# helenypzhang/Subspace-Multimodal-Learning

Measured on AMD Instinct MI355X. Metric: bags/sec fwd+bwd, DeformCrossTransMIL N=10k x 512, higher is better.
Workload: dtype f32

## Files before the change

include/smml.h:

```cpp
#ifndef SMML_H_
#define SMML_H_

#include <stddef.h>

#ifdef __cplusplus
extern "C" {
#endif

const char* smml_last_error(void);
int smml_abi_version(void);
int smml_device_check(int device);
void* smml_event_create(void);
int smml_event_destroy(void* ev);
int smml_event_record(void* ev, void* stream);
int smml_event_elapsed_ms(void* start, void* stop, float* ms);

int smml_gemm_f32(const float* A, const float* B, float* C, const float* bias, const float* residual,
                  int M, int N, int K, long long sam, long long sak, long long sbk, long long sbn,
                  long long ldc, long long ldr, int nb0, int nb1, long long sa0, long long sa1,
                  long long sb0, long long sb1, long long sc0, long long sc1, long long sbias0,
                  long long sbias1, int bias_mode, int rows_per_bias, long long bias_ld, int act,
                  int splitk, int accumulate, float alpha, float beta, void* stream);
void smml_gemm_force_generic(int on);
void smml_gemm_set_mode(int mode);
int smml_gemm_get_mode(void);
void smml_gemm_set_small_tile(int v);

int smml_gemm_b16(const void* A, const void* B, void* C, const float* bias, int M, int N, int K, long long lda, long long ldb,
                  long long ldc, int trans, int out_bf16, int splitk, void* stream);
void smml_gemm_b16_set_tile(int mode);
void smml_gemm_b16_set_slice_major(int on);
int smml_gemm_b16_batched(const void* A, const void* B, void* C, const float* bias, int M, int N, int K, long long lda, long long ldb,
                          long long ldc, int trans, int out_bf16, int splitk, int nb, long long sa, long long sb, long long sc, void* stream);

int smml_layernorm_fwd_f32(const float* x, const float* gamma, const float* beta, float* y, float* mean,
                           float* rstd, long long R, int C, float eps, void* stream);
int smml_layernorm_bwd_f32(const float* x, const float* dy, const float* gamma, const float* mean,
                           const float* rstd, float* dx, float* dgamma, float* dbeta, long long R, int C,
                           long long rows_per_dy, float dy_scale, int accumulate_dx, void* stream);

int smml_colsum_f32(const float* x, float* out, int nb, long long R, int C, float scale, void* stream);

int smml_orth_loss_f32(const float* P, const float* Ph, const float* G, const float* Gh, const float* dloss, float* loss,
                       float* dP, float* dPh, float* dG, float* dGh, int B, int D, float gamma, void* stream);

int smml_batchloss_tail_f32(const float* go, const float* gv, const float* dloss, float* loss, float* dgo, float* dgv, int R, int nv,
                            float n_total, void* stream);

int smml_relu_bwd_f32(const float* dy, const float* y, float* dx, long long n, void* stream);

int smml_offsets_out_len(int s, int ks, int r);
int smml_offsets_fwd_f32(const float* q, const float* w0, const float* b0, const float* w2, float* vgrid,
                         float* vs, int B, int Hh, int Ww, int G, int dg, int ks, int r, int posdim,
                         float offset_scale, void* stream);
size_t smml_offsets_bwd_workspace_bytes(int B, int Hh, int Ww, int G, int dg, int ks, int r, int posdim);
// ... 208 lines not shown
```

subspace-multimodal-learning_amd/_capi.py:

```python
from __future__ import annotations

import ctypes as C
import os
from typing import Optional

import torch

_PKG = os.path.dirname(os.path.abspath(__file__))
LIB_PATH = os.environ.get("SMML_LIB") or os.path.join(_PKG, "lib", "libsmml_hip.so")

_f = C.c_void_p


class DeformOpts(C.Structure):
    _fields_ = [("seed_offset", C.c_void_p), ("raw_distance", C.c_int), ("mask_table", C.c_void_p), ("mask_table_pmax", C.c_float),
                ("export_masks", C.c_void_p), ("region_lds_cap", C.c_int)]


_o = C.POINTER(DeformOpts)
_i, _ll, _fl, _sz = C.c_int, C.c_longlong, C.c_float, C.c_size_t

ABI_VERSION = 2

SIGNATURES = {
    "smml_last_error": (C.c_char_p, []),
    "smml_abi_version": (_i, []),
    "smml_device_check": (_i, [_i]),
    "smml_gemm_f32": (_i, [_f, _f, _f, _f, _f, _i, _i, _i, _ll, _ll, _ll, _ll, _ll, _ll, _i, _i, _ll, _ll, _ll, _ll,
                           _ll, _ll, _ll, _ll, _i, _i, _ll, _i, _i, _i, _fl, _fl, _f]),
    "smml_gemm_force_generic": (None, [_i]),
    "smml_gemm_set_mode": (None, [_i]),
    "smml_gemm_get_mode": (_i, []),
    "smml_gemm_set_small_tile": (None, [_i]),
    "smml_gemm_b16": (_i, [_f, _f, _f, _f, _i, _i, _i, _ll, _ll, _ll, _i, _i, _i, _f]),
    "smml_gemm_b16_set_tile": (None, [_i]),
    "smml_gemm_b16_set_slice_major": (None, [_i]),
    "smml_gemm_b16_batched": (_i, [_f, _f, _f, _f, _i, _i, _i, _ll, _ll, _ll, _i, _i, _i, _i, _ll, _ll, _ll, _f]),
    "smml_attn16_fwd_workspace_bytes": (_sz, [_i, _i, _i]),
    "smml_attn16_fwd_f32": (_i, [_f, _f, _f, _f, _f, _f, _sz, _i, _i, _i, _i, _fl, _i, _i, _i, _f]),
    "smml_attn16_set_fewkeys": (None, [_i]),
    "smml_attn16_set_query_blocks": (None, [_i]),
    "smml_attn16_fwd_b16": (_i, [_f, _f, _f, _f, _f, _f, _f, _sz, _i, _i, _i, _i, _fl, _i, _ll, _ll, _ll, _ll, _ll, _ll, _f]),
    "smml_attn16_bwd_b16": (_i, [_f] * 11 + [_sz, _i, _i, _i, _i, _fl, _i] + [_ll] * 9 + [_i, _f]),
    "smml_attn16_bwd_workspace_bytes": (_sz, [_i, _i, _i]),
    "smml_attn16_bwd_f32": (_i, [_f] * 10 + [_f, _sz, _i, _i, _i, _i, _fl, _i, _i, _f]),
    "smml_layernorm_fwd_f32": (_i, [_f, _f, _f, _f, _f, _f, _ll, _i, _fl, _f]),
    "smml_layernorm_bwd_f32": (_i, [_f, _f, _f, _f, _f, _f, _f, _f, _ll, _i, _ll, _fl, _i, _f]),
    "smml_colsum_f32": (_i, [_f, _f, _i, _ll, _i, _fl, _f]),
    "smml_orth_loss_f32": (_i, [_f] * 10 + [_i, _i, _fl, _f]),
    "smml_batchloss_tail_f32": (_i, [_f, _f, _f, _f, _f, _f, _i, _i, _fl, _f]),
    "smml_relu_bwd_f32": (_i, [_f, _f, _f, _ll, _f]),
    "smml_offsets_out_len": (_i, [_i, _i, _i]),
    "smml_offsets_fwd_f32": (_i, [_f, _f, _f, _f, _f, _f, _i, _i, _i, _i, _i, _i, _i, _i, _fl, _f]),
    "smml_offsets_bwd_workspace_bytes": (_sz, [_i, _i, _i, _i, _i, _i, _i, _i]),
    "smml_offsets_bwd_f32": (_i, [_f, _f, _f, _f, _f, _f, _f, _f, _f, _f, _f, _sz, _i, _i, _i, _i, _i, _i, _i, _i, _fl, _i, _f]),
    "smml_bilinear_sample_fwd_f32": (_i, [_f, _f, _f, _i, _i, _i, _i, _i, _i, _i, _f]),
    "smml_bilinear_sample_bwd_f32": (_i, [_f, _f, _f, _f, _f, _i, _i, _i, _i, _i, _i, _i, _f]),
    "smml_bilinear_corners_f32": (_i, [_f, _f, _f, _f, _i, _i, _i, _i, _f]),
    "smml_deform_attn_nst": (_i, [_i]),
    "smml_deform_attn_fwd_f32": (_i, [_f] * 15 + [_i, _i, _i, _i, _i, _i, _fl, _fl, C.c_ulonglong, _f, _f, _f] + [_o]),
    "smml_deform_attn_dropout_mask_f32": (_i, [_f, _i, _i, _i, _i, _fl, C.c_ulonglong, _f] + [_o]),
    "smml_deform_attn_relu1_masks": (_i, [_f, _f, _f, _f, _f, _i, _i, _i, _i, _i, _f] + [_o]),
# ... 118 lines not shown
```

subspace-multimodal-learning_amd/csrc/gemm.hip:

```cpp
#include "smml_common.h"
#include <atomic>

namespace {

constexpr int BM = 128, BN = 64, BK = 16;
constexpr int LDA = BM + 4, LDB = BN + 4;

struct GemmArgs {
  const float* A; const float* B; float* C; const float* bias; const float* residual;
  int M, N, K;
  long long sam, sak, sbk, sbn, ldc, ldr;
  int nb0, nb1;
  long long sa0, sa1, sb0, sb1, sc0, sc1, sbias0, sbias1;
  int bias_mode, rows_per_bias; long long bias_ld;
  int act, splitk; float alpha, beta;
  int atomic;
  int swap_xy;
};

__device__ __forceinline__ float apply_act(float v, int act) {
  if (act == 1) return fmaxf(v, 0.f);
  if (act == 2) return tanhf(v);
  return v;
}

__global__ __launch_bounds__(256) void gemm_f32_kernel(GemmArgs g) {
  __shared__ float As[BK][LDA];
  __shared__ float Bs[BK][LDB];
  const int tid = threadIdx.x, wave = tid >> 6, lane = tid & 63, c = lane & 31, hf = lane >> 5;
  const int zb = blockIdx.z / g.splitk, ks = blockIdx.z - zb * g.splitk;
  const int b0 = zb / g.nb1, b1 = zb - b0 * g.nb1;
  const float* A = g.A + b0 * g.sa0 + b1 * g.sa1;
  const float* B = g.B + b0 * g.sb0 + b1 * g.sb1;
  float* C = g.C + b0 * g.sc0 + b1 * g.sc1;
  const int m0 = (g.swap_xy ? blockIdx.y : blockIdx.x) * BM, n0 = (g.swap_xy ? blockIdx.x : blockIdx.y) * BN;
  const int ktiles = (g.K + BK - 1) / BK;
  const int tps = (ktiles + g.splitk - 1) / g.splitk;
  const int kt0 = ks * tps, kt1 = min(ktiles, kt0 + tps);

  floatx16 acc0 = {0}, acc1 = {0};
  const bool a_kcontig = (g.sak == 1);
  const bool b_kcontig = (g.sbk == 1) && (g.sbn != 1);

  for (int kt = kt0; kt < kt1; ++kt) {
    const int k0 = kt * BK;
    __syncthreads();
    if (a_kcontig) {
      const int k = tid & 15;
#pragma unroll
      for (int i = 0; i < 8; ++i) {
// ... 30 lines not shown
    __syncthreads();
#pragma unroll
    for (int st = 0; st < BK / 2; ++st) {
      const float a = As[2 * st + hf][wave * 32 + c];
      acc0 = mfma32(a, Bs[2 * st + hf][c], acc0);
      acc1 = mfma32(a, Bs[2 * st + hf][32 + c], acc1);
    }
  }

  const float* bias = g.bias ? g.bias + b0 * g.sbias0 + b1 * g.sbias1 : nullptr;
  const float* res = g.residual ? g.residual + b0 * g.sc0 + b1 * g.sc1 : nullptr;
#pragma unroll
  for (int t = 0; t < 2; ++t) {
    const int n = n0 + 32 * t + c;
    if (n >= g.N) continue;
#pragma unroll
    for (int r = 0; r < 16; ++r) {
      const int m = m0 + wave * 32 + acc_row(r, hf);
      if (m >= g.M) continue;
      float v = g.alpha * (t == 0 ? acc0[r] : acc1[r]);
      if (g.atomic) {
        if (bias && ks == 0) v += (g.bias_mode == 2) ? bias[(m / g.rows_per_bias) * g.bias_ld + n] : bias[n];
        atomicAdd(&C[m * g.ldc + n], v);
      } else {
        if (bias) v += (g.bias_mode == 2) ? bias[(m / g.rows_per_bias) * g.bias_ld + n] : bias[n];
        v = apply_act(v, g.act);
        if (res) v = fmaf(g.beta, res[m * g.ldr + n], v);
        C[m * g.ldc + n] = v;
      }
    }
  }
}

template <int BN_, bool A_KC, bool B_KC, int FBM = 128>
__global__ __launch_bounds__(256, 2) void gemm_f32_fast_kernel(GemmArgs g) {
  constexpr int FBK = 16, NI = BN_ / 64, MI = FBM / 64;
  constexpr int NA = FBM / 64;
  constexpr int A_LD = A_KC ? (FBK + 4) : (FBM + 4);
  constexpr int B_LD = B_KC ? (FBK + 4) : (BN_ + 4);
  __shared__ __attribute__((aligned(16))) float As[(A_KC ? FBM : FBK) * A_LD];
  __shared__ __attribute__((aligned(16))) float Bs[(B_KC ? BN_ : FBK) * B_LD];
  const int tid = threadIdx.x, wave = tid >> 6, lane = tid & 63, c = lane & 31, hf = lane >> 5;
  const int wm = wave >> 1, wn = wave & 1;
  const int zb = blockIdx.z / g.splitk, ks = blockIdx.z - zb * g.splitk;
  const int b0 = zb / g.nb1, b1 = zb - b0 * g.nb1;
  const float* A = g.A + b0 * g.sa0 + b1 * g.sa1;
  const float* B = g.B + b0 * g.sb0 + b1 * g.sb1;
  float* C = g.C + b0 * g.sc0 + b1 * g.sc1;
  const int m0 = (g.swap_xy ? blockIdx.y : blockIdx.x) * FBM, n0 = (g.swap_xy ? blockIdx.x : blockIdx.y) * BN_;
  const int ktiles = (g.K + FBK - 1) / FBK;
  const int tps = (ktiles + g.splitk - 1) / g.splitk;
  const int kt0 = ks * tps, kt1 = min(ktiles, kt0 + tps);

  float4 ra[NA], rb[NI];
  const float* pa[NA];
  const float* pb[NI];
  int ka[NA], kb_[NI];
  int fa[NA], fb[NI];
  constexpr int MQ = FBM / 4;
#pragma unroll
  for (int i = 0; i < NA; ++i) {
    if (A_KC) {
      const int row = (tid >> 2) + 64 * i, kq = tid & 3;
      pa[i] = A + (long long)min(m0 + row, g.M - 1) * g.sam + 4 * kq;
      ka[i] = 4 * kq; fa[i] = 1;
    } else {
      const int idx = tid + 256 * i, k = idx / MQ, mq = idx - k * MQ, gm = m0 + 4 * mq;
      pa[i] = A + min(gm, g.M - 1);
      ka[i] = k; fa[i] = (gm >= g.M) ? 0 : (gm + 3 < g.M ? 1 : 2);
    }
  }
#pragma unroll
  for (int i = 0; i < NI; ++i) {
    if (B_KC) {
      const int row = (tid >> 2) + 64 * i, kq = tid & 3;
      pb[i] = B + (long long)min(n0 + row, g.N - 1) * g.sbn + 4 * kq;
      kb_[i] = 4 * kq; fb[i] = 1;
    } else {
      constexpr int NQ = BN_ / 4;
      const int idx = tid + 256 * i, k = idx / NQ, nq = idx - k * NQ, gn = n0 + 4 * nq;
      pb[i] = B + min(gn, g.N - 1);
      kb_[i] = k; fb[i] = (gn >= g.N) ? 0 : (gn + 3 < g.N ? 1 : 2);
    }
  }
  auto load_tile = [&](int kt) {
    const int k0 = kt * FBK;
#pragma unroll
    for (int i = 0; i < NA; ++i) {
      if (A_KC) {
        ra[i] = (k0 + ka[i] < g.K) ? *reinterpret_cast<const float4*>(pa[i] + k0) : make_float4(0.f, 0.f, 0.f, 0.f);
      } else {
        const int k = k0 + ka[i];
        const float* p = pa[i] + (long long)min(k, g.K - 1) * g.sak;
        if (k >= g.K || fa[i] == 0) ra[i] = make_float4(0.f, 0.f, 0.f, 0.f);
        else if (fa[i] == 1) ra[i] = *reinterpret_cast<const float4*>(p);
        else { const int gm = m0 + 4 * ((tid + 256 * i) % MQ), last = g.M - 1 - gm;
               ra[i] = make_float4(p[0], p[min(1, last)], p[min(2, last)], p[min(3, last)]); }
      }
    }
#pragma unroll
    for (int i = 0; i < NI; ++i) {
      if (B_KC) {
        rb[i] = (k0 + kb_[i] < g.K) ? *reinterpret_cast<const float4*>(pb[i] + k0) : make_float4(0.f, 0.f, 0.f, 0.f);
      } else {
        const int k = k0 + kb_[i];
        const float* p = pb[i] + (long long)min(k, g.K - 1) * g.sbk;
        if (k >= g.K || fb[i] == 0) rb[i] = make_float4(0.f, 0.f, 0.f, 0.f);
        else if (fb[i] == 1) rb[i] = *reinterpret_cast<const float4*>(p);
        else { constexpr int NQ = BN_ / 4; const int idx = tid + 256 * i, gn = n0 + 4 * (idx - (idx / NQ) * NQ), last = g.N - 1 - gn;
               rb[i] = make_float4(p[0], p[min(1, last)], p[min(2, last)], p[min(3, last)]); }
      }
    }
  };
  auto store_tile = [&]() {
#pragma unroll
    for (int i = 0; i < NA; ++i) {
      if (A_KC) { const int row = (tid >> 2) + 64 * i, kq = tid & 3; *reinterpret_cast<float4*>(&As[row * A_LD + 4 * kq]) = ra[i]; }
      else { const int idx = tid + 256 * i, k = idx / MQ, mq = idx - k * MQ; *reinterpret_cast<float4*>(&As[k * A_LD + 4 * mq]) = ra[i]; }
    }
#pragma unroll
    for (int i = 0; i < NI; ++i) {
      if (B_KC) { const int row = (tid >> 2) + 64 * i, kq = tid & 3; *reinterpret_cast<float4*>(&Bs[row * B_LD + 4 * kq]) = rb[i]; }
      else { constexpr int NQ = BN_ / 4; const int idx = tid + 256 * i, k = idx / NQ, nq = idx - k * NQ;
             *reinterpret_cast<float4*>(&Bs[k * B_LD + 4 * nq]) = rb[i]; }
    }
  };

  floatx16 acc[MI][NI];
#pragma unroll
  for (int mi = 0; mi < MI; ++mi)
#pragma unroll
    for (int ni = 0; ni < NI; ++ni) acc[mi][ni] = floatx16{0};

  if (kt0 < kt1) load_tile(kt0);
  for (int kt = kt0; kt < kt1; ++kt) {
    __syncthreads();
    store_tile();
    __syncthreads();
    if (kt + 1 < kt1) load_tile(kt + 1);
    float af[MI][8], bf[NI][8];
#pragma unroll
    for (int mi = 0; mi < MI; ++mi) {
      const int row = wm * (FBM / 2) + mi * 32 + c;
      if (A_KC) {
        const float4 x = *reinterpret_cast<const float4*>(&As[row * A_LD + 8 * hf]);
        const float4 y = *reinterpret_cast<const float4*>(&As[row * A_LD + 8 * hf + 4]);
        af[mi][0] = x.x; af[mi][1] = x.y; af[mi][2] = x.z; af[mi][3] = x.w;
        af[mi][4] = y.x; af[mi][5] = y.y; af[mi][6] = y.z; af[mi][7] = y.w;
      } else {
#pragma unroll
        for (int st = 0; st < 8; ++st) af[mi][st] = As[(8 * hf + st) * A_LD + row];
      }
    }
#pragma unroll
    for (int ni = 0; ni < NI; ++ni) {
      const int col = wn * (BN_ / 2) + ni * 32 + c;
      if (B_KC) {
        const float4 x = *reinterpret_cast<const float4*>(&Bs[col * B_LD + 8 * hf]);
        const float4 y = *reinterpret_cast<const float4*>(&Bs[col * B_LD + 8 * hf + 4]);
        bf[ni][0] = x.x; bf[ni][1] = x.y; bf[ni][2] = x.z; bf[ni][3] = x.w;
        bf[ni][4] = y.x; bf[ni][5] = y.y; bf[ni][6] = y.z; bf[ni][7] = y.w;
      } else {
#pragma unroll
        for (int st = 0; st < 8; ++st) bf[ni][st] = Bs[(8 * hf + st) * B_LD + col];
      }
    }
#pragma unroll
    for (int st = 0; st < 8; ++st)
#pragma unroll
      for (int mi = 0; mi < MI; ++mi)
#pragma unroll
        for (int ni = 0; ni < NI; ++ni) acc[mi][ni] = mfma32(af[mi][st], bf[ni][st], acc[mi][ni]);
  }

  const float* bias = g.bias ? g.bias + b0 * g.sbias0 + b1 * g.sbias1 : nullptr;
  const float* res = g.residual ? g.residual + b0 * g.sc0 + b1 * g.sc1 : nullptr;
  if (!g.atomic && m0 + FBM <= g.M && n0 + BN_ <= g.N) {
#pragma unroll
    for (int mi = 0; mi < MI; ++mi)
#pragma unroll
      for (int ni = 0; ni < NI; ++ni) {
        const int n = n0 + wn * (BN_ / 2) + ni * 32 + c;
        const int mb = m0 + wm * (FBM / 2) + mi * 32;
        float rv[16];
#pragma unroll
        for (int r = 0; r < 16; ++r) rv[r] = res ? res[(long long)(mb + acc_row(r, hf)) * g.ldr + n] : 0.f;
#pragma unroll
        for (int r = 0; r < 16; ++r) {
          const int m = mb + acc_row(r, hf);
          float v = g.alpha * acc[mi][ni][r];
          if (bias) v += (g.bias_mode == 2) ? bias[(m / g.rows_per_bias) * g.bias_ld + n] : bias[n];
          v = apply_act(v, g.act);
          C[(long long)m * g.ldc + n] = fmaf(g.beta, rv[r], v);
        }
      }
    return;
  }
#pragma unroll
  for (int mi = 0; mi < MI; ++mi)
#pragma unroll
    for (int ni = 0; ni < NI; ++ni) {
      const int n = n0 + wn * (BN_ / 2) + ni * 32 + c;
      if (n >= g.N) continue;
#pragma unroll
      for (int r = 0; r < 16; ++r) {
// ... 199 lines not shown
  for (int mi = 0; mi < MI; ++mi)
#pragma unroll
    for (int ni = 0; ni < NI; ++ni) {
      const int n = n0 + wn * (BN_ / 2) + ni * 32 + c;
      if (n >= g.N) continue;
#pragma unroll
      for (int r = 0; r < 16; ++r) {
        const int m = m0 + wm * (FBM / 2) + mi * 32 + acc_row(r, hf);
        if (m >= g.M) continue;
        float v = g.alpha * acc[mi][ni][r];
        if (g.atomic) {
          if (bias && ks == 0) v += (g.bias_mode == 2) ? bias[(m / g.rows_per_bias) * g.bias_ld + n] : bias[n];
          atomicAdd(&C[m * g.ldc + n], v);
        } else {
          if (bias) v += (g.bias_mode == 2) ? bias[(m / g.rows_per_bias) * g.bias_ld + n] : bias[n];
          v = apply_act(v, g.act);
          if (res) v = fmaf(g.beta, res[m * g.ldr + n], v);
          C[m * g.ldc + n] = v;
        }
      }
    }
}

}

static std::atomic<int> g_force_generic{0};
static std::atomic<int> g_mode{0};
extern "C" void smml_gemm_force_generic(int on) { g_force_generic = on; }
extern "C" void smml_gemm_set_mode(int mode) { g_mode = mode; }
extern "C" int smml_gemm_get_mode(void) { return g_mode; }
static std::atomic<int> g_small_tile{0};
extern "C" void smml_gemm_set_small_tile(int v) { g_small_tile = v; }

extern "C" int smml_gemm_f32(const float* A, const float* B, float* C, const float* bias, const float* residual,
                             int M, int N, int K, long long sam, long long sak, long long sbk, long long sbn,
                             long long ldc, long long ldr, int nb0, int nb1, long long sa0, long long sa1,
                             long long sb0, long long sb1, long long sc0, long long sc1, long long sbias0,
                             long long sbias1, int bias_mode, int rows_per_bias, long long bias_ld, int act,
                             int splitk, int accumulate, float alpha, float beta, void* stream) {
  SMML_REQUIRE(A && B && C, "smml_gemm_f32: null operand");
  SMML_REQUIRE(M > 0 && N > 0 && K > 0 && nb0 > 0 && nb1 > 0, "smml_gemm_f32: non-positive size (M=%d N=%d K=%d)", M, N, K);
  SMML_REQUIRE(splitk >= 1, "smml_gemm_f32: splitk must be >= 1");
  const int atomic = (splitk > 1 || accumulate) ? 1 : 0;
  SMML_REQUIRE(!(atomic && (act != 0 || residual)), "smml_gemm_f32: split-K / accumulate excludes activation/residual");
  SMML_REQUIRE(bias_mode >= 0 && bias_mode <= 2, "smml_gemm_f32: bad bias_mode %d", bias_mode);
  SMML_REQUIRE(bias_mode != 2 || rows_per_bias > 0, "smml_gemm_f32: rows_per_bias must be positive");
  SMML_REQUIRE(act >= 0 && act <= 2, "smml_gemm_f32: bad activation %d", act);
  const long long gz = (long long)nb0 * nb1 * splitk;
  const long long gy = (N + BN - 1) / BN, gx = (M + BM - 1) / BM;
  const int swap_xy = gy > 65535;
  SMML_REQUIRE(gz <= 65535 && (swap_xy ? gx : gy) <= 65535,
               "smml_gemm_f32: grid too large (batch*splitk=%lld, row tiles=%lld, col tiles=%lld)", gz, gx, gy);
  GemmArgs g{A, B, C, bias_mode ? bias : nullptr, residual, M, N, K, sam, sak, sbk, sbn, ldc, ldr, nb0, nb1,
             sa0, sa1, sb0, sb1, sc0, sc1, sbias0, sbias1, bias_mode, rows_per_bias > 0 ? rows_per_bias : 1,
             bias_ld, act, splitk, alpha, beta, atomic, swap_xy};
  SMML_REQUIRE(!bias_mode || bias, "smml_gemm_f32: bias_mode set but bias is null");
  auto al4 = [](long long v) { return (v & 3) == 0; };
  auto al16 = [](const void* p) { return (((size_t)p) & 15) == 0; };
  const bool a_kc = (sak == 1), a_mc = (sam == 1 && sak != 1);
  const bool b_kc = (sbk == 1 && sbn != 1), b_nc = (sbn == 1);
  const bool a_ok = al16(A) && al4(sa0) && al4(sa1) && ((a_kc && al4(sam)) || (a_mc && al4(sak)));
  const bool b_ok = al16(B) && al4(sb0) && al4(sb1) && ((b_kc && al4(sbn)) || (b_nc && al4(sbk)));
  const bool k_ok = (!a_kc && !b_kc) || (K % 4) == 0;
  if (a_ok && b_ok && k_ok && !g_force_generic) {
    const int bn = (N > 64 && gx * ((N + 127) / 128) * gz >= 1024) ? 128 : 64;
    const long long fy = (N + bn - 1) / bn;
    const bool small = bn == 64 && M > 64 && (g_small_tile == 2 || (g_small_tile == 0 && gx * fy * gz < 512));
    const long long fx = small ? (M + 63) / 64 : gx;
    const int fswap = fy > 65535;
    SMML_REQUIRE((fswap ? fx : fy) <= 65535, "smml_gemm_f32: grid too large");
    g.swap_xy = fswap;
    dim3 grid((unsigned)(fswap ? fy : fx), (unsigned)(fswap ? fx : fy), (unsigned)gz);
    hipStream_t st = (hipStream_t)stream;
    const bool bf3 = (g_mode == 2) || (g_mode == 0 && K >= 2048 && M >= 1024 && N >= 1024);
    const bool bf1 = (g_mode == 3), f1 = (g_mode == 4);
#define SMML_FAST(BNV, AK, BK2)                                                                   \
  do {                                                                                            \
    if (f1) hipLaunchKernelGGL((gemm_bf3_kernel<BNV, AK, BK2, 1, 128, true>), grid, dim3(256), 0, st, g); \
    else if (bf1) hipLaunchKernelGGL((gemm_bf3_kernel<BNV, AK, BK2, 1>), grid, dim3(256), 0, st, g);   \
    else if (bf3) hipLaunchKernelGGL((gemm_bf3_kernel<BNV, AK, BK2>), grid, dim3(256), 0, st, g); \
    else hipLaunchKernelGGL((gemm_f32_fast_kernel<BNV, AK, BK2>), grid, dim3(256), 0, st, g);     \
  } while (0)
#define SMML_SMALL(AK, BK2)                                                                          \
  do {                                                                                               \
    if (f1) hipLaunchKernelGGL((gemm_bf3_kernel<64, AK, BK2, 1, 64, true>), grid, dim3(256), 0, st, g);   \
    else if (bf1) hipLaunchKernelGGL((gemm_bf3_kernel<64, AK, BK2, 1, 64>), grid, dim3(256), 0, st, g);   \
    else if (bf3) hipLaunchKernelGGL((gemm_bf3_kernel<64, AK, BK2, 3, 64>), grid, dim3(256), 0, st, g); \
    else hipLaunchKernelGGL((gemm_f32_fast_kernel<64, AK, BK2, 64>), grid, dim3(256), 0, st, g);     \
  } while (0)
    if (small) {
      if (a_kc && b_kc) SMML_SMALL(true, true); else if (a_kc) SMML_SMALL(true, false);
      else if (b_kc) SMML_SMALL(false, true); else SMML_SMALL(false, false);
    } else if (bn == 128) {
      if (a_kc && b_kc) SMML_FAST(128, true, true); else if (a_kc) SMML_FAST(128, true, false);
      else if (b_kc) SMML_FAST(128, false, true); else SMML_FAST(128, false, false);
    } else {
      if (a_kc && b_kc) SMML_FAST(64, true, true); else if (a_kc) SMML_FAST(64, true, false);
      else if (b_kc) SMML_FAST(64, false, true); else SMML_FAST(64, false, false);
    }
#undef SMML_FAST
#undef SMML_SMALL
    SMML_LAUNCH_CHECK("smml_gemm_f32/fast");
    return SMML_OK;
  }
  dim3 grid((unsigned)(swap_xy ? gy : gx), (unsigned)(swap_xy ? gx : gy), (unsigned)gz);
  hipLaunchKernelGGL(gemm_f32_kernel, grid, dim3(256), 0, (hipStream_t)stream, g);
  SMML_LAUNCH_CHECK("smml_gemm_f32");
  return SMML_OK;
}
```

subspace-multimodal-learning_amd/functional.py:

```python
from __future__ import annotations

import math
import os
from typing import Optional

import ctypes as C_

import torch

from . import _capi as capi

ACT_NONE, ACT_RELU, ACT_TANH = 0, 1, 2


class KernelTimer:

    def __init__(self):
        self.enabled = False
        self.pairs = {"deform_attn_fwd": [], "cpb_bwd": []}
        self.work = {"deform_attn_fwd": [], "cpb_bwd": []}

    def events(self, name, pairs_count):
        if not self.enabled:
            return None, None
# ... 56 lines not shown
            n *= d
        if (n == 0 or n > self.LIMIT or torch.device(device).type != "cuda" or not self.enabled
                or torch.cuda.is_current_stream_capturing()):
            return torch.zeros(shape, device=device, dtype=torch.float32)
        key = torch.device(device).index if torch.device(device).index is not None else torch.cuda.current_device()
        buf, used = self.slabs.get(key, (None, self.SLAB))
        n4 = (n + 3) & ~3
        if used + n4 > self.SLAB:
            buf, used = torch.zeros(self.SLAB, device=device, dtype=torch.float32), 0
        self.slabs[key] = (buf, used + n4)
        return buf[used:used + n].view(shape)


_ZEROS = _ZeroPool()


def _zeros_like(t: torch.Tensor) -> torch.Tensor:
    return _ZEROS.zeros(t.shape, t.device)


def _c(t: torch.Tensor) -> torch.Tensor:
    if t.dtype != torch.float32:
        t = t.float()
    return t if t.is_contiguous() else t.contiguous()


def _gemm(A, B, C, *, M, N, K, sam, sak, sbk, sbn, ldc, bias=None, bias_mode=0, rows_per_bias=1, bias_ld=0,
          residual=None, ldr=0, act=ACT_NONE, splitk=1, alpha=1.0, nb0=1, nb1=1, sa0=0, sa1=0, sb0=0, sb1=0,
          sc0=0, sc1=0, sbias0=0, sbias1=0, beta=1.0, accumulate=0):
    capi.check(capi.lib().smml_gemm_f32(
        capi.fptr(A), capi.fptr(B), capi.fptr(C), capi.fptr(bias), capi.fptr(residual), M, N, K,
        sam, sak, sbk, sbn, ldc, ldr, nb0, nb1, sa0, sa1, sb0, sb1, sc0, sc1, sbias0, sbias1,
        bias_mode, rows_per_bias, bias_ld, act, splitk, accumulate, float(alpha), float(beta), capi.stream()), "gemm")


class _prec:

    def __init__(self, mode):
        self.mode = int(mode or 0)

    def __enter__(self):
        if self.mode:
            L = capi.lib()
            self.prev = L.smml_gemm_get_mode()
            L.smml_gemm_set_mode(self.mode)

    def __exit__(self, *a):
        if self.mode:
            capi.lib().smml_gemm_set_mode(self.prev)


def _splitk_for(out_rows: int, out_cols: int, k: int, batches: int = 1) -> int:
    tiles = ((out_rows + 127) // 128) * ((out_cols + 63) // 64) * batches
    want = max(1, 1024 // max(tiles, 1))
    return int(max(1, min(want, (k + 255) // 256, 65535 // max(batches, 1))))


def colsum(x2d_or_3d: torch.Tensor, scale: float = 1.0) -> torch.Tensor:
    x = x2d_or_3d
    nb, R, Cc = x.shape
    out = _ZEROS.zeros((nb, Cc), x.device)
    capi.check(capi.lib().smml_colsum_f32(capi.fptr(x), capi.fptr(out), nb, R, Cc, float(scale), capi.stream()), "colsum")
    return out


class _Linear(torch.autograd.Function):
    @staticmethod
    def forward(ctx, x, weight, bias, act, rows_per_bias, residual, prec=0):
        x = _c(x); weight = _c(weight)
        ctx.prec = 3 if prec == 4 else prec
        K = x.shape[-1]
        M = x.numel() // K
        N = weight.shape[0]
        y = torch.empty(*x.shape[:-1], N, device=x.device, dtype=torch.float32)
        bias_mode = 0
        if bias is not None:
            bias = _c(bias)
            bias_mode = 2 if bias.dim() == 2 else 1
        res = _c(residual) if residual is not None else None
        with _prec(prec):
            _gemm(x, weight, y, M=M, N=N, K=K, sam=K, sak=1, sbk=1, sbn=K, ldc=N, bias=bias, bias_mode=bias_mode,
                  rows_per_bias=rows_per_bias, bias_ld=N, residual=res, ldr=N, act=act)
        ctx.act, ctx.rows_per_bias, ctx.bias_mode = act, rows_per_bias, bias_mode
        ctx.has_res = residual is not None
        ctx.save_for_backward(x, weight, y if act != ACT_NONE else None)
        return y

    @staticmethod
    def backward(ctx, dy):
        x, weight, y = ctx.saved_tensors
        dy = _c(dy)
        K = x.shape[-1]
        M = x.numel() // K
        N = weight.shape[0]
        dres = dy if ctx.has_res else None
        if ctx.act == ACT_RELU:
            dpre = torch.empty_like(dy)
            capi.check(capi.lib().smml_relu_bwd_f32(capi.fptr(dy), capi.fptr(y), capi.fptr(dpre), dy.numel(),
                                                    capi.stream()), "relu_bwd")
        elif ctx.act == ACT_TANH:
            dpre = dy * (1.0 - y * y)
        else:
            dpre = dy
        dx = dw = db = None
        with _prec(ctx.prec):
            if ctx.needs_input_grad[0]:
                dx = torch.empty_like(x)
                _gemm(dpre, weight, dx, M=M, N=K, K=N, sam=N, sak=1, sbk=K, sbn=1, ldc=K)
            if ctx.needs_input_grad[1]:
                dw = _zeros_like(weight)
                _gemm(dpre, x, dw, M=N, N=K, K=M, sam=1, sak=N, sbk=K, sbn=1, ldc=K, splitk=_splitk_for(N, K, M))
        if ctx.bias_mode and ctx.needs_input_grad[2]:
            if ctx.bias_mode == 1:
                db = colsum(dpre.reshape(1, M, N))[0]
            else:
                db = colsum(dpre.reshape(M // ctx.rows_per_bias, ctx.rows_per_bias, N))
        return dx, dw, db, None, None, dres, None


def linear(x, weight, bias=None, act: int = ACT_NONE, rows_per_bias: int = 1, residual=None, prec: int = 0):
    return _Linear.apply(x, weight, bias, act, rows_per_bias, residual, prec)


class _DualLinearRelu(torch.autograd.Function):
    @staticmethod
    def forward(ctx, x, w0, b0, w1, b1):
        x = _c(x)
        K = x.shape[-1]
        M = x.numel() // K
        N = w0.shape[0]
        w = torch.stack((_c(w0), _c(w1)))
        b = torch.stack((_c(b0), _c(b1)))
        y = torch.empty(2, *x.shape[:-1], N, device=x.device, dtype=torch.float32)
        _gemm(x, w, y, M=M, N=N, K=K, sam=K, sak=1, sbk=1, sbn=K, ldc=N, bias=b, bias_mode=1, act=ACT_RELU, nb1=2, sa1=0,
              sb1=N * K, sc1=M * N, sbias1=N)
        ctx.save_for_backward(x, y)
        return y[0], y[1]

    @staticmethod
    def backward(ctx, dy0, dy1):
        x, y = ctx.saved_tensors
        K = x.shape[-1]
        M = x.numel() // K
        N = y.shape[-1]
        L = capi.lib()
        dpre = torch.empty_like(y)
        for i, dy in enumerate((dy0, dy1)):
            capi.check(L.smml_relu_bwd_f32(capi.fptr(_c(dy)), capi.fptr(y[i]), capi.fptr(dpre[i]), dy.numel(), capi.stream()), "relu_bwd")
        dx = None
        if ctx.needs_input_grad[0]:
            raise RuntimeError("dual_linear_relu: the shared input is a bag of features (no gradient path is built)")
        dw = _ZEROS.zeros((2, N, K), x.device)
        _gemm(dpre, x, dw, M=N, N=K, K=M, sam=1, sak=N, sbk=K, sbn=1, ldc=K, nb1=2, sa1=M * N, sb1=0, sc1=N * K,
              splitk=_splitk_for(N, K, M, 2))
        db = colsum(dpre.reshape(2, M, N))
        return dx, dw[0], db[0], dw[1], db[1]


def dual_linear_relu(x, w0, b0, w1, b1):
    return _DualLinearRelu.apply(x, w0, b0, w1, b1)


def _bptr(t: torch.Tensor):
    if t.dtype != torch.bfloat16:
        raise RuntimeError(f"smml bf16 kernel got dtype {t.dtype}")
    return capi.ptr(t)


def gemm_b16(A, B, C, *, M, N, K, lda, ldb, ldc, trans=False, bias=None, splitk=1, nb=1, sa=0, sb=0, sc=0, a_off=0, b_off=0, c_off=0):
    if C.dtype not in (torch.bfloat16, torch.float32):
        raise RuntimeError(f"gemm_b16: output dtype {C.dtype}")
    _bptr(A), _bptr(B), capi.ptr(C)
    pa = C_.c_void_p(A.data_ptr() + 2 * a_off)
    pb = C_.c_void_p(B.data_ptr() + 2 * b_off)
    pc = C_.c_void_p(C.data_ptr() + C.element_size() * c_off)
    capi.check(capi.lib().smml_gemm_b16_batched(pa, pb, pc, capi.fptr(bias), M, N, K, lda, ldb, ldc, int(trans),
                                                int(C.dtype == torch.bfloat16), splitk, nb, sa, sb, sc, capi.stream()), "gemm_b16")


class _LinearB16(torch.autograd.Function):
    @staticmethod
    def forward(ctx, x, weight, bias, out_bf16, skip):
        if x.dtype != torch.bfloat16:
            raise RuntimeError("linear_b16: x must be bf16 (the caller casts once)")
        x = x if x.is_contiguous() else x.contiguous()
        wb = weight.detach().to(torch.bfloat16)
        K = x.shape[-1]
        N = weight.shape[0]
        if skip:
# ... 1398 lines not shown
```

Measured before the change: 1205.

## Fuse ReLU-backward gating and bias column sums into weight-gradient GEMM

Adds an extended fp32 GEMM entry point whose TN kernel masks the A operand by a ReLU gate while loading tiles and accumulates per-row sums of A for the bias gradient. Linear and dual-linear ReLU backward use it when the input gradient is not needed, skipping the separate relu_bwd pass, the dpre buffer and the colsum kernel. It also picks split-K automatically from the CU count. In exchange it adds an extra gate load per tile and atomic adds for the column sums, and the dual path now stacks dy0/dy1 into a new tensor.

```diff
diff --git a/include/smml.h b/include/smml.h
--- a/include/smml.h
+++ b/include/smml.h
@@ -21,6 +21,12 @@
                   long long sb0, long long sb1, long long sc0, long long sc1, long long sbias0,
                   long long sbias1, int bias_mode, int rows_per_bias, long long bias_ld, int act,
                   int splitk, int accumulate, float alpha, float beta, void* stream);
+int smml_gemm_f32_ex(const float* A, const float* B, float* C, const float* bias, const float* residual,
+                     int M, int N, int K, long long sam, long long sak, long long sbk, long long sbn,
+                     long long ldc, long long ldr, int nb0, int nb1, long long sa0, long long sa1,
+                     long long sb0, long long sb1, long long sc0, long long sc1, long long sbias0,
+                     long long sbias1, int bias_mode, int rows_per_bias, long long bias_ld, int act,
+                     int splitk, int accumulate, float alpha, float beta, const float* a_gate, float* a_colsum, void* stream);
 void smml_gemm_force_generic(int on);
 void smml_gemm_set_mode(int mode);
 int smml_gemm_get_mode(void);
diff --git a/subspace-multimodal-learning_amd/_capi.py b/subspace-multimodal-learning_amd/_capi.py
--- a/subspace-multimodal-learning_amd/_capi.py
+++ b/subspace-multimodal-learning_amd/_capi.py
@@ -28,6 +28,8 @@
     "smml_device_check": (_i, [_i]),
     "smml_gemm_f32": (_i, [_f, _f, _f, _f, _f, _i, _i, _i, _ll, _ll, _ll, _ll, _ll, _ll, _i, _i, _ll, _ll, _ll, _ll,
                            _ll, _ll, _ll, _ll, _i, _i, _ll, _i, _i, _i, _fl, _fl, _f]),
+    "smml_gemm_f32_ex": (_i, [_f, _f, _f, _f, _f, _i, _i, _i, _ll, _ll, _ll, _ll, _ll, _ll, _i, _i, _ll, _ll, _ll, _ll,
+                              _ll, _ll, _ll, _ll, _i, _i, _ll, _i, _i, _i, _fl, _fl, _f, _f, _f]),
     "smml_gemm_force_generic": (None, [_i]),
     "smml_gemm_set_mode": (None, [_i]),
     "smml_gemm_get_mode": (_i, []),
diff --git a/subspace-multimodal-learning_amd/csrc/gemm.hip b/subspace-multimodal-learning_amd/csrc/gemm.hip
--- a/subspace-multimodal-learning_amd/csrc/gemm.hip
+++ b/subspace-multimodal-learning_amd/csrc/gemm.hip
@@ -1,4 +1,5 @@
 #include "smml_common.h"
+#include <algorithm>
 #include <atomic>
 
 namespace {
@@ -16,6 +17,8 @@
   int act, splitk; float alpha, beta;
   int atomic;
   int swap_xy;
+  const float* gate;
+  float* asum;
 };
 
 __device__ __forceinline__ float apply_act(float v, int act) {
@@ -112,10 +115,12 @@
   }
 }
 
-template <int BN_, bool A_KC, bool B_KC, int FBM = 128>
+template <int BN_, bool A_KC, bool B_KC, int FBM = 128, bool EX = false>
 __global__ __launch_bounds__(256, 2) void gemm_f32_fast_kernel(GemmArgs g) {
   constexpr int FBK = 16, NI = BN_ / 64, MI = FBM / 64;
-  constexpr int NA = FBM / 64;
+  constexpr int NA = FBM * FBK / 1024, NB = BN_ * FBK / 1024;
+  constexpr int KQ = FBK / 4, RP = 256 / KQ;
+  static_assert(!EX || (!A_KC && !B_KC), "gate / column sums of A: the TN (weight-gradient) form only");
   constexpr int A_LD = A_KC ? (FBK + 4) : (FBM + 4);
   constexpr int B_LD = B_KC ? (FBK + 4) : (BN_ + 4);
   __shared__ __attribute__((aligned(16))) float As[(A_KC ? FBM : FBK) * A_LD];
@@ -127,21 +132,22 @@
   const float* A = g.A + b0 * g.sa0 + b1 * g.sa1;
   const float* B = g.B + b0 * g.sb0 + b1 * g.sb1;
   float* C = g.C + b0 * g.sc0 + b1 * g.sc1;
+  const float* Gt = (EX && g.gate) ? g.gate + b0 * g.sa0 + b1 * g.sa1 : nullptr;
   const int m0 = (g.swap_xy ? blockIdx.y : blockIdx.x) * FBM, n0 = (g.swap_xy ? blockIdx.x : blockIdx.y) * BN_;
   const int ktiles = (g.K + FBK - 1) / FBK;
   const int tps = (ktiles + g.splitk - 1) / g.splitk;
   const int kt0 = ks * tps, kt1 = min(ktiles, kt0 + tps);
 
-  float4 ra[NA], rb[NI];
+  float4 ra[NA], rb[NB];
   const float* pa[NA];
-  const float* pb[NI];
-  int ka[NA], kb_[NI];
-  int fa[NA], fb[NI];
+  const float* pb[NB];
+  int ka[NA], kb_[NB];
+  int fa[NA], fb[NB];
   constexpr int MQ = FBM / 4;
 #pragma unroll
   for (int i = 0; i < NA; ++i) {
     if (A_KC) {
-      const int row = (tid >> 2) + 64 * i, kq = tid & 3;
+      const int row = tid / KQ + RP * i, kq = tid % KQ;
       pa[i] = A + (long long)min(m0 + row, g.M - 1) * g.sam + 4 * kq;
       ka[i] = 4 * kq; fa[i] = 1;
     } else {
@@ -151,9 +157,9 @@
     }
   }
 #pragma unroll
-  for (int i = 0; i < NI; ++i) {
+  for (int i = 0; i < NB; ++i) {
     if (B_KC) {
-      const int row = (tid >> 2) + 64 * i, kq = tid & 3;
+      const int row = tid / KQ + RP * i, kq = tid % KQ;
       pb[i] = B + (long long)min(n0 + row, g.N - 1) * g.sbn + 4 * kq;
       kb_[i] = 4 * kq; fb[i] = 1;
     } else {
@@ -176,10 +182,17 @@
         else if (fa[i] == 1) ra[i] = *reinterpret_cast<const float4*>(p);
         else { const int gm = m0 + 4 * ((tid + 256 * i) % MQ), last = g.M - 1 - gm;
                ra[i] = make_float4(p[0], p[min(1, last)], p[min(2, last)], p[min(3, last)]); }
-      }
-    }
-#pragma unroll
-    for (int i = 0; i < NI; ++i) {
+        if (EX && Gt && k < g.K && fa[i] != 0) {
+          const float* q = Gt + (p - A);
+          float4 gv;
+          if (fa[i] == 1) gv = *reinterpret_cast<const float4*>(q);
+          else { const int last = g.M - 1 - (m0 + 4 * ((tid + 256 * i) % MQ)); gv = make_float4(q[0], q[min(1, last)], q[min(2, last)], q[min(3, last)]); }
+          ra[i] = make_float4(gv.x > 0.f ? ra[i].x : 0.f, gv.y > 0.f ? ra[i].y : 0.f, gv.z > 0.f ? ra[i].z : 0.f, gv.w > 0.f ? ra[i].w : 0.f);
+        }
+      }
+    }
+#pragma unroll
+    for (int i = 0; i < NB; ++i) {
       if (B_KC) {
         rb[i] = (k0 + kb_[i] < g.K) ? *reinterpret_cast<const float4*>(pb[i] + k0) : make_float4(0.f, 0.f, 0.f, 0.f);
       } else {
@@ -195,12 +208,12 @@
   auto store_tile = [&]() {
 #pragma unroll
     for (int i = 0; i < NA; ++i) {
-      if (A_KC) { const int row = (tid >> 2) + 64 * i, kq = tid & 3; *reinterpret_cast<float4*>(&As[row * A_LD + 4 * kq]) = ra[i]; }
+      if (A_KC) { const int row = tid / KQ + RP * i, kq = tid % KQ; *reinterpret_cast<float4*>(&As[row * A_LD + 4 * kq]) = ra[i]; }
       else { const int idx = tid + 256 * i, k = idx / MQ, mq = idx - k * MQ; *reinterpret_cast<float4*>(&As[k * A_LD + 4 * mq]) = ra[i]; }
     }
 #pragma unroll
-    for (int i = 0; i < NI; ++i) {
-      if (B_KC) { const int row = (tid >> 2) + 64 * i, kq = tid & 3; *reinterpret_cast<float4*>(&Bs[row * B_LD + 4 * kq]) = rb[i]; }
+    for (int i = 0; i < NB; ++i) {
+      if (B_KC) { const int row = tid / KQ + RP * i, kq = tid % KQ; *reinterpret_cast<float4*>(&Bs[row * B_LD + 4 * kq]) = rb[i]; }
       else { constexpr int NQ = BN_ / 4; const int idx = tid + 256 * i, k = idx / NQ, nq = idx - k * NQ;
              *reinterpret_cast<float4*>(&Bs[k * B_LD + 4 * nq]) = rb[i]; }
     }
@@ -211,46 +224,72 @@
   for (int mi = 0; mi < MI; ++mi)
 #pragma unroll
     for (int ni = 0; ni < NI; ++ni) acc[mi][ni] = floatx16{0};
+
+  const bool do_sum = EX && g.asum && n0 == 0;
+  float4 sa[NA];
+#pragma unroll
+  for (int i = 0; i < NA; ++i) sa[i] = make_float4(0.f, 0.f, 0.f, 0.f);
 
   if (kt0 < kt1) load_tile(kt0);
   for (int kt = kt0; kt < kt1; ++kt) {
     __syncthreads();
     store_tile();
+    if (do_sum) {
+#pragma unroll
+      for (int i = 0; i < NA; ++i) { sa[i].x += ra[i].x; sa[i].y += ra[i].y; sa[i].z += ra[i].z; sa[i].w += ra[i].w; }
+    }
     __syncthreads();
     if (kt + 1 < kt1) load_tile(kt + 1);
-    float af[MI][8], bf[NI][8];
-#pragma unroll
-    for (int mi = 0; mi < MI; ++mi) {
-      const int row = wm * (FBM / 2) + mi * 32 + c;
-      if (A_KC) {
-        const float4 x = *reinterpret_cast<const float4*>(&As[row * A_LD + 8 * hf]);
-        const float4 y = *reinterpret_cast<const float4*>(&As[row * A_LD + 8 * hf + 4]);
-        af[mi][0] = x.x; af[mi][1] = x.y; af[mi][2] = x.z; af[mi][3] = x.w;
-        af[mi][4] = y.x; af[mi][5] = y.y; af[mi][6] = y.z; af[mi][7] = y.w;
-      } else {
-#pragma unroll
-        for (int st = 0; st < 8; ++st) af[mi][st] = As[(8 * hf + st) * A_LD + row];
-      }
-    }
-#pragma unroll
-    for (int ni = 0; ni < NI; ++ni) {
-      const int col = wn * (BN_ / 2) + ni * 32 + c;
-      if (B_KC) {
-        const float4 x = *reinterpret_cast<const float4*>(&Bs[col * B_LD + 8 * hf]);
-        const float4 y = *reinterpret_cast<const float4*>(&Bs[col * B_LD + 8 * hf + 4]);
-        bf[ni][0] = x.x; bf[ni][1] = x.y; bf[ni][2] = x.z; bf[ni][3] = x.w;
-        bf[ni][4] = y.x; bf[ni][5] = y.y; bf[ni][6] = y.z; bf[ni][7] = y.w;
-      } else {
-#pragma unroll
-        for (int st = 0; st < 8; ++st) bf[ni][st] = Bs[(8 * hf + st) * B_LD + col];
-      }
-    }
-#pragma unroll
-    for (int st = 0; st < 8; ++st)
-#pragma unroll
-      for (int mi = 0; mi < MI; ++mi)
-#pragma unroll
-        for (int ni = 0; ni < NI; ++ni) acc[mi][ni] = mfma32(af[mi][st], bf[ni][st], acc[mi][ni]);
+#pragma unroll
+    for (int sub = 0; sub < FBK / 16; ++sub) {
+      float af[MI][8], bf[NI][8];
+#pragma unroll
+      for (int mi = 0; mi < MI; ++mi) {
+        const int row = wm * (FBM / 2) + mi * 32 + c;
+        if (A_KC) {
+          const float4 x = *reinterpret_cast<const float4*>(&As[row * A_LD + 16 * sub + 8 * hf]);
+          const float4 y = *reinterpret_cast<const float4*>(&As[row * A_LD + 16 * sub + 8 * hf + 4]);
+          af[mi][0] = x.x; af[mi][1] = x.y; af[mi][2] = x.z; af[mi][3] = x.w;
+          af[mi][4] = y.x; af[mi][5] = y.y; af[mi][6] = y.z; af[mi][7] = y.w;
+        } else {
+#pragma unroll
+          for (int st = 0; st < 8; ++st) af[mi][st] = As[(16 * sub + 8 * hf + st) * A_LD + row];
+        }
+      }
+#pragma unroll
+      for (int ni = 0; ni < NI; ++ni) {
+        const int col = wn * (BN_ / 2) + ni * 32 + c;
+        if (B_KC) {
+          const float4 x = *reinterpret_cast<const float4*>(&Bs[col * B_LD + 16 * sub + 8 * hf]);
+          const float4 y = *reinterpret_cast<const float4*>(&Bs[col * B_LD + 16 * sub + 8 * hf + 4]);
+          bf[ni][0] = x.x; bf[ni][1] = x.y; bf[ni][2] = x.z; bf[ni][3] = x.w;
+          bf[ni][4] = y.x; bf[ni][5] = y.y; bf[ni][6] = y.z; bf[ni][7] = y.w;
+        } else {
+#pragma unroll
+          for (int st = 0; st < 8; ++st) bf[ni][st] = Bs[(16 * sub + 8 * hf + st) * B_LD + col];
+        }
+      }
+#pragma unroll
+      for (int st = 0; st < 8; ++st)
+#pragma unroll
+        for (int mi = 0; mi < MI; ++mi)
+#pragma unroll
+          for (int ni = 0; ni < NI; ++ni) acc[mi][ni] = mfma32(af[mi][st], bf[ni][st], acc[mi][ni]);
+    }
+  }
+  if (EX) {
+    if (do_sum) {
+      __syncthreads();
+#pragma unroll
+      for (int i = 0; i < NA; ++i) { const int idx = tid + 256 * i, k = idx / MQ, mq = idx - k * MQ; *reinterpret_cast<float4*>(&As[k * A_LD + 4 * mq]) = sa[i]; }
+      __syncthreads();
+      if (tid < FBM && m0 + tid < g.M) {
+        float t = 0.f;
+#pragma unroll
+        for (int k = 0; k < FBK; ++k) t += As[k * A_LD + tid];
+        atomicAdd(&g.asum[(long long)zb * g.M + m0 + tid], t);
+      }
+    }
   }
 
   const float* bias = g.bias ? g.bias + b0 * g.sbias0 + b1 * g.sbias1 : nullptr;
@@ -516,28 +555,42 @@
 static std::atomic<int> g_small_tile{0};
 extern "C" void smml_gemm_set_small_tile(int v) { g_small_tile = v; }
 
-extern "C" int smml_gemm_f32(const float* A, const float* B, float* C, const float* bias, const float* residual,
-                             int M, int N, int K, long long sam, long long sak, long long sbk, long long sbn,
-                             long long ldc, long long ldr, int nb0, int nb1, long long sa0, long long sa1,
-                             long long sb0, long long sb1, long long sc0, long long sc1, long long sbias0,
-                             long long sbias1, int bias_mode, int rows_per_bias, long long bias_ld, int act,
-                             int splitk, int accumulate, float alpha, float beta, void* stream) {
+static int resident_slots() {
+  static std::atomic<int> cus{0};
+  int n = cus;
+  if (n == 0) {
+    int dev = 0, v = 0;
+    if (hipGetDevice(&dev) != hipSuccess || hipDeviceGetAttribute(&v, hipDeviceAttributeMultiprocessorCount, dev) != hipSuccess || v <= 0) v = 256;
+    cus = n = v;
+  }
+  return 2 * n;
+}
+
+static int gemm_launch(const float* A, const float* B, float* C, const float* bias, const float* residual,
+                       int M, int N, int K, long long sam, long long sak, long long sbk, long long sbn,
+                       long long ldc, long long ldr, int nb0, int nb1, long long sa0, long long sa1,
+                       long long sb0, long long sb1, long long sc0, long long sc1, long long sbias0,
+                       long long sbias1, int bias_mode, int rows_per_bias, long long bias_ld, int act,
+                       int splitk, int accumulate, float alpha, float beta, const float* a_gate, float* a_colsum, bool extended, void* stream) {
   SMML_REQUIRE(A && B && C, "smml_gemm_f32: null operand");
   SMML_REQUIRE(M > 0 && N > 0 && K > 0 && nb0 > 0 && nb1 > 0, "smml_gemm_f32: non-positive size (M=%d N=%d K=%d)", M, N, K);
+  const bool ex = a_gate || a_colsum;
+  const bool auto_split = extended && splitk == 0;
+  if (auto_split) splitk = 1;
   SMML_REQUIRE(splitk >= 1, "smml_gemm_f32: splitk must be >= 1");
-  const int atomic = (splitk > 1 || accumulate) ? 1 : 0;
+  const int atomic = (splitk > 1 || accumulate || auto_split) ? 1 : 0;
   SMML_REQUIRE(!(atomic && (act != 0 || residual)), "smml_gemm_f32: split-K / accumulate excludes activation/residual");
   SMML_REQUIRE(bias_mode >= 0 && bias_mode <= 2, "smml_gemm_f32: bad bias_mode %d", bias_mode);
   SMML_REQUIRE(bias_mode != 2 || rows_per_bias > 0, "smml_gemm_f32: rows_per_bias must be positive");
   SMML_REQUIRE(act >= 0 && act <= 2, "smml_gemm_f32: bad activation %d", act);
-  const long long gz = (long long)nb0 * nb1 * splitk;
+  long long gz = (long long)nb0 * nb1 * splitk;
   const long long gy = (N + BN - 1) / BN, gx = (M + BM - 1) / BM;
   const int swap_xy = gy > 65535;
   SMML_REQUIRE(gz <= 65535 && (swap_xy ? gx : gy) <= 65535,
                "smml_gemm_f32: grid too large (batch*splitk=%lld, row tiles=%lld, col tiles=%lld)", gz, gx, gy);
   GemmArgs g{A, B, C, bias_mode ? bias : nullptr, residual, M, N, K, sam, sak, sbk, sbn, ldc, ldr, nb0, nb1,
              sa0, sa1, sb0, sb1, sc0, sc1, sbias0, sbias1, bias_mode, rows_per_bias > 0 ? rows_per_bias : 1,
-             bias_ld, act, splitk, alpha, beta, atomic, swap_xy};
+             bias_ld, act, splitk, alpha, beta, atomic, swap_xy, a_gate, a_colsum};
   SMML_REQUIRE(!bias_mode || bias, "smml_gemm_f32: bias_mode set but bias is null");
   auto al4 = [](long long v) { return (v & 3) == 0; };
   auto al16 = [](const void* p) { return (((size_t)p) & 15) == 0; };
@@ -546,16 +599,28 @@
   const bool a_ok = al16(A) && al4(sa0) && al4(sa1) && ((a_kc && al4(sam)) || (a_mc && al4(sak)));
   const bool b_ok = al16(B) && al4(sb0) && al4(sb1) && ((b_kc && al4(sbn)) || (b_nc && al4(sbk)));
   const bool k_ok = (!a_kc && !b_kc) || (K % 4) == 0;
-  if (a_ok && b_ok && k_ok && !g_force_generic) {
+  const bool fast = a_ok && b_ok && k_ok && !g_force_generic;
+  if (ex) {
+    SMML_REQUIRE(fast && a_mc && b_nc && g_mode <= 1, "smml_gemm_f32_ex: gate / column sums need the exact-fp32 tiled TN form "
+                 "(A(m,k) and B(k,n) with unit stride on m / n, 16-byte aligned, other strides multiples of 4)");
+    SMML_REQUIRE(!a_gate || al16(a_gate), "smml_gemm_f32_ex: gate must be 16-byte aligned");
+  }
+  if (fast) {
+    hipStream_t st = (hipStream_t)stream;
+    if (auto_split) {
+      const long long nbat = (long long)nb0 * nb1, tiles = gx * gy * nbat;
+      long long sk = std::max<long long>(1, 2LL * resident_slots() / std::max<long long>(tiles, 1));
+      sk = std::min<long long>(std::min<long long>(sk, ((long long)K + 255) / 256), std::max<long long>(1, 65535 / nbat));
+      g.splitk = (int)sk; gz = nbat * sk;
+    }
     const int bn = (N > 64 && gx * ((N + 127) / 128) * gz >= 1024) ? 128 : 64;
     const long long fy = (N + bn - 1) / bn;
-    const bool small = bn == 64 && M > 64 && (g_small_tile == 2 || (g_small_tile == 0 && gx * fy * gz < 512));
+    const bool small = !ex && bn == 64 && M > 64 && (g_small_tile == 2 || (g_small_tile != 1 && gx * fy * gz < 512));
     const long long fx = small ? (M + 63) / 64 : gx;
     const int fswap = fy > 65535;
     SMML_REQUIRE((fswap ? fx : fy) <= 65535, "smml_gemm_f32: grid too large");
     g.swap_xy = fswap;
     dim3 grid((unsigned)(fswap ? fy : fx), (unsigned)(fswap ? fx : fy), (unsigned)gz);
-    hipStream_t st = (hipStream_t)stream;
     const bool bf3 = (g_mode == 2) || (g_mode == 0 && K >= 2048 && M >= 1024 && N >= 1024);
     const bool bf1 = (g_mode == 3), f1 = (g_mode == 4);
 #define SMML_FAST(BNV, AK, BK2)                                                                   \
@@ -572,7 +637,10 @@
     else if (bf3) hipLaunchKernelGGL((gemm_bf3_kernel<64, AK, BK2, 3, 64>), grid, dim3(256), 0, st, g); \
     else hipLaunchKernelGGL((gemm_f32_fast_kernel<64, AK, BK2, 64>), grid, dim3(256), 0, st, g);     \
   } while (0)
-    if (small) {
+    if (ex) {
+      if (bn == 128) hipLaunchKernelGGL((gemm_f32_fast_kernel<128, false, false, 128, true>), grid, dim3(256), 0, st, g);
+      else hipLaunchKernelGGL((gemm_f32_fast_kernel<64, false, false, 128, true>), grid, dim3(256), 0, st, g);
+    } else if (small) {
       if (a_kc && b_kc) SMML_SMALL(true, true); else if (a_kc) SMML_SMALL(true, false);
       else if (b_kc) SMML_SMALL(false, true); else SMML_SMALL(false, false);
     } else if (bn == 128) {
@@ -592,3 +660,24 @@
   SMML_LAUNCH_CHECK("smml_gemm_f32");
   return SMML_OK;
 }
+
+extern "C" int smml_gemm_f32(const float* A, const float* B, float* C, const float* bias, const float* residual,
+                             int M, int N, int K, long long sam, long long sak, long long sbk, long long sbn,
+                             long long ldc, long long ldr, int nb0, int nb1, long long sa0, long long sa1,
+                             long long sb0, long long sb1, long long sc0, long long sc1, long long sbias0,
+                             long long sbias1, int bias_mode, int rows_per_bias, long long bias_ld, int act,
+                             int splitk, int accumulate, float alpha, float beta, void* stream) {
+  return gemm_launch(A, B, C, bias, residual, M, N, K, sam, sak, sbk, sbn, ldc, ldr, nb0, nb1, sa0, sa1, sb0, sb1, sc0, sc1, sbias0, sbias1,
+                     bias_mode, rows_per_bias, bias_ld, act, splitk, accumulate, alpha, beta, nullptr, nullptr, false, stream);
+}
+
+extern "C" int smml_gemm_f32_ex(const float* A, const float* B, float* C, const float* bias, const float* residual,
+                                int M, int N, int K, long long sam, long long sak, long long sbk, long long sbn,
+                                long long ldc, long long ldr, int nb0, int nb1, long long sa0, long long sa1,
+                                long long sb0, long long sb1, long long sc0, long long sc1, long long sbias0,
+                                long long sbias1, int bias_mode, int rows_per_bias, long long bias_ld, int act,
+                                int splitk, int accumulate, float alpha, float beta, const float* a_gate, float* a_colsum, void* stream) {
+  SMML_REQUIRE(splitk >= 0, "smml_gemm_f32_ex: splitk must be >= 0");
+  return gemm_launch(A, B, C, bias, residual, M, N, K, sam, sak, sbk, sbn, ldc, ldr, nb0, nb1, sa0, sa1, sb0, sb1, sc0, sc1, sbias0, sbias1,
+                     bias_mode, rows_per_bias, bias_ld, act, splitk, accumulate, alpha, beta, a_gate, a_colsum, true, stream);
+}
diff --git a/subspace-multimodal-learning_amd/functional.py b/subspace-multimodal-learning_amd/functional.py
--- a/subspace-multimodal-learning_amd/functional.py
+++ b/subspace-multimodal-learning_amd/functional.py
@@ -112,6 +112,20 @@
         capi.fptr(A), capi.fptr(B), capi.fptr(C), capi.fptr(bias), capi.fptr(residual), M, N, K,
         sam, sak, sbk, sbn, ldc, ldr, nb0, nb1, sa0, sa1, sb0, sb1, sc0, sc1, sbias0, sbias1,
         bias_mode, rows_per_bias, bias_ld, act, splitk, accumulate, float(alpha), float(beta), capi.stream()), "gemm")
+
+
+def _gemm_ex(A, B, C, *, M, N, K, sam, sak, sbk, sbn, ldc, splitk=0, gate=None, a_colsum=None, nb1=1, sa1=0, sb1=0, sc1=0):
+    capi.check(capi.lib().smml_gemm_f32_ex(
+        capi.fptr(A), capi.fptr(B), capi.fptr(C), None, None, M, N, K, sam, sak, sbk, sbn, ldc, 0, 1, nb1, 0, sa1, 0, sb1, 0, sc1, 0, 0,
+        0, 1, 0, ACT_NONE, splitk, 0, 1.0, 1.0, capi.fptr(gate), capi.fptr(a_colsum), capi.stream()), "gemm_ex")
+
+
+def _wgrad_ex_ok(dy, x, prec: int = 0) -> bool:
+    N, K = dy.shape[-1], x.shape[-1]
+    M = x.numel() // K
+    if prec or capi.lib().smml_gemm_get_mode() > 1 or (N & 3) or (K & 3) or (dy.data_ptr() & 15) or (x.data_ptr() & 15):
+        return False
+    return not (M >= 2048 and N >= 1024 and K >= 1024)
 
 
 class _prec:
@@ -174,7 +188,12 @@
         M = x.numel() // K
         N = weight.shape[0]
         dres = dy if ctx.has_res else None
-        if ctx.act == ACT_RELU:
+        want_dw, want_db = ctx.needs_input_grad[1], bool(ctx.bias_mode) and ctx.needs_input_grad[2]
+        ex = want_dw and ctx.act != ACT_TANH and _wgrad_ex_ok(dy, x, ctx.prec)
+        gate = None
+        if ctx.act == ACT_RELU and ex and not ctx.needs_input_grad[0]:
+            dpre, gate = dy, y
+        elif ctx.act == ACT_RELU:
             dpre = torch.empty_like(dy)
             capi.check(capi.lib().smml_relu_bwd_f32(capi.fptr(dy), capi.fptr(y), capi.fptr(dpre), dy.numel(),
                                                     capi.stream()), "relu_bwd")
@@ -187,10 +206,18 @@
             if ctx.needs_input_grad[0]:
                 dx = torch.empty_like(x)
                 _gemm(dpre, weight, dx, M=M, N=K, K=N, sam=N, sak=1, sbk=K, sbn=1, ldc=K)
-            if ctx.needs_input_grad[1]:
+            if want_dw and ex:
+                dw = _zeros_like(weight)
+                if want_db and ctx.bias_mode == 1:
+                    db = _ZEROS.zeros((N,), x.device)
+                _gemm_ex(dpre, x, dw, M=N, N=K, K=M, sam=1, sak=N, sbk=K, sbn=1, ldc=K, gate=gate, a_colsum=db)
+            elif want_dw:
                 dw = _zeros_like(weight)
                 _gemm(dpre, x, dw, M=N, N=K, K=M, sam=1, sak=N, sbk=K, sbn=1, ldc=K, splitk=_splitk_for(N, K, M))
-        if ctx.bias_mode and ctx.needs_input_grad[2]:
+        if want_db and db is None:
+            if gate is not None:
+                dpre = torch.empty_like(dy)
+                capi.check(capi.lib().smml_relu_bwd_f32(capi.fptr(dy), capi.fptr(y), capi.fptr(dpre), dy.numel(), capi.stream()), "relu_bwd")
             if ctx.bias_mode == 1:
                 db = colsum(dpre.reshape(1, M, N))[0]
             else:
@@ -224,17 +251,21 @@
         M = x.numel() // K
         N = y.shape[-1]
         L = capi.lib()
+        if ctx.needs_input_grad[0]:
+            raise RuntimeError("dual_linear_relu: the shared input is a bag of features (no gradient path is built)")
+        dw = _ZEROS.zeros((2, N, K), x.device)
+        if dy0.dtype == dy1.dtype == torch.float32 and _wgrad_ex_ok(y, x):
+            dy = torch.stack((dy0, dy1))
+            db = _ZEROS.zeros((2, N), x.device)
+            _gemm_ex(dy, x, dw, M=N, N=K, K=M, sam=1, sak=N, sbk=K, sbn=1, ldc=K, nb1=2, sa1=M * N, sb1=0, sc1=N * K, gate=y, a_colsum=db)
+            return None, dw[0], db[0], dw[1], db[1]
         dpre = torch.empty_like(y)
         for i, dy in enumerate((dy0, dy1)):
             capi.check(L.smml_relu_bwd_f32(capi.fptr(_c(dy)), capi.fptr(y[i]), capi.fptr(dpre[i]), dy.numel(), capi.stream()), "relu_bwd")
-        dx = None
-        if ctx.needs_input_grad[0]:
-            raise RuntimeError("dual_linear_relu: the shared input is a bag of features (no gradient path is built)")
-        dw = _ZEROS.zeros((2, N, K), x.device)
         _gemm(dpre, x, dw, M=N, N=K, K=M, sam=1, sak=N, sbk=K, sbn=1, ldc=K, nb1=2, sa1=M * N, sb1=0, sc1=N * K,
               splitk=_splitk_for(N, K, M, 2))
         db = colsum(dpre.reshape(2, M, N))
-        return dx, dw[0], db[0], dw[1], db[1]
+        return None, dw[0], db[0], dw[1], db[1]
 
 
 def dual_linear_relu(x, w0, b0, w1, b1):
```

Result: no change. 1203, median of 2 (-0.2%).
